# YuliangXiu/ICON

Hardware: NVIDIA H100
Metric: M query-points/sec at 256^3 grid (higher is better)
Workload: dtype f32

## Files before the change

### icon_b200/csrc/common.cuh

```cuda
#pragma once
#include <cuda_runtime.h>
#include <stdint.h>
#include <stdio.h>

#include "../../include/icon_b200.h"

namespace icon {

void set_error(const char *fmt, ...);
void count_launch(int n = 1);

#define ICON_CHECK_ARG(cond, ...)                 \
    do {                                          \
        if (!(cond)) {                            \
            icon::set_error(__VA_ARGS__);         \
            return ICON_EINVAL;                   \
        }                                         \
    } while (0)

#define ICON_CUDA(expr)                                                              \
    do {                                                                             \
        cudaError_t _e = (expr);                                                     \
        if (_e != cudaSuccess) {                                                     \
            icon::set_error("%s:%d %s -> %s", __FILE__, __LINE__, #expr,             \
// ... 124 lines not shown
    int nlevels;
    int lvl_cnt[TREE_MAX_LEVELS];
    int lvl_off[TREE_MAX_LEVELS];
};

struct MeshView : FaceTree {
    const float4 *tri;
    const float4 *sph;
    const float4 *attr;
    const float4 *rbox;
    float *vnormals;
    void *vn_ws;
    unsigned long long *keys;
    int32_t *rcount;
    int32_t *roff;
    int32_t *rlist;
    MeshHeader *hdr;
    void *scan_ws;
    float4 *bxyz;
    int32_t *bperm;
    float *brec;
    int32_t *bface;
    float *bub;
    int32_t *foff;
    unsigned short *flist;
    float *fkey;
    int64_t face_cap;
    int V;
};
size_t mesh_ws_bytes(int V, int F);
MeshView mesh_view(const void *ws, int V, int F);
void bricks_forget(const MeshView &m);

void profile_mark(int i, cudaStream_t stream);

size_t scan_ws_bytes(int64_t n);
int scan_exclusive_i32(const int32_t *in, int32_t *out, int64_t n, int64_t *d_total ,
                       void *ws, cudaStream_t stream);

struct CsrWs {
    int32_t *cnt, *cursor;
    void *scan_ws;
};
CsrWs csr_take(Carver &c, int64_t rows);
int csr_build(const int32_t *own, const int32_t *key, int64_t n, int R, int32_t *off, int32_t *list, int32_t *ucnt,
              const CsrWs &w, cudaStream_t stream);

size_t vertex_corners_ws_bytes(int V, int F);
int vertex_corners(const int64_t *faces, int F, int V, int32_t *off, int32_t *list, void *ws, cudaStream_t stream);

template <class Fn>
__device__ __forceinline__ void for_each_pass_corner(const int32_t *corners, int n, Fn &&fn) {
    for (int pass = 0; pass < 3; ++pass) {
        const int c = (pass + 1) % 3;
        for (int i = 0; i < n; ++i)
            if (corners[i] % 3 == c) fn(corners[i] / 3, c);
    }
}

size_t area_vertex_normals_ws_bytes(int V, int F);
int area_vertex_normals(const float *verts, int V, const int64_t *faces, int F, float *out, void *ws,
                        cudaStream_t stream);

}
```

### icon_b200/csrc/mlp.cu

```cuda
#include "common.cuh"
#include "query_common.cuh"

namespace icon {

constexpr int MP = 64;
constexpr int MT = 256;
constexpr int KC = 16;

constexpr int OFF_W0 = 0;
constexpr int OFF_B0 = OFF_W0 + 16 * 512;
constexpr int OFF_W1 = OFF_B0 + 512;
constexpr int OFF_B1 = OFF_W1 + 512 * 256;
constexpr int OFF_W2 = OFF_B1 + 256;
constexpr int OFF_B2 = OFF_W2 + 272 * 128;
constexpr int OFF_W3 = OFF_B2 + 128;
constexpr int OFF_B3 = OFF_W3 + 144;
static_assert(OFF_B3 + 1 == ICON_MLP_PACKED_FLOATS, "packed layout");

template <int MODE>
__global__ void __launch_bounds__(MT, 2) k_query_mlp(QueryParams q) {
    extern __shared__ __align__(16) float sm[];
    float *x0s = sm;
    float *stage = sm + 16 * MP;
    float *h1s = stage + 10240;
// ... 9 lines not shown

    {
        const float4 *src = (const float4 *)(W + OFF_W1);
        for (int i = tid; i < KC * 256 / 4; i += MT) cp_async16(w1c + 4 * i, src + i);
        cp_async_commit();
    }

    {
        const int pl = tid & (MP - 1), grp = tid >> 6;
        const int64_t pi = p0 + pl;
        const bool live = pi < q.N;
        if (MODE == 3) {
            for (int r = grp; r < 16; r += 4) x0s[r * MP + pl] = (live && r < c0) ? q.raw[(size_t)r * q.N + pi] : 0.f;
        } else {
            float4 xyz = live ? q.xyz4[pi] : make_float4(0.f, 0.f, 0.f, 0.f);
            if (MODE == 0) {
                const bool has_vis = q.feats & ICON_FEAT_VIS;
                const int d = has_vis ? q.C / 2 : q.C;
                float4 r0 = make_float4(0.f, 0.f, 0.f, 0.f), r1 = r0;
                if (live) {
                    const float4 *r = (const float4 *)(q.rec + 8 * pi);
                    r0 = r[0]; r1 = r[1];
                }
                const float vis = r1.w;
                if (grp == 0) {
                    float sdf = r0.x, cx = r0.y, cy = r0.z, cz = r0.w;
                    const bool outlier = live && fabsf(sdf) >= q.clip;
                    if (outlier) sdf = sdf > 0.f ? 1.f : -1.f;
                    int col = d;
                    x0s[col++ * MP + pl] = sdf;
                    if (q.feats & ICON_FEAT_CMAP) {
                        if (outlier) {
                            long long K = *q.d_K;
                            long long k3 = 3ll * (long long)q.krank[pi];
                            cx = (float)q.signs[(k3) % K];
                            cy = (float)q.signs[(k3 + 1) % K];
                            cz = (float)q.signs[(k3 + 2) % K];
                        }
                        x0s[col++ * MP + pl] = cx;
                        x0s[col++ * MP + pl] = cy;
                        x0s[col++ * MP + pl] = cz;
                    }
                    if (q.feats & ICON_FEAT_NORM) {
                        x0s[col++ * MP + pl] = r1.x;
                        x0s[col++ * MP + pl] = r1.y;
                        x0s[col++ * MP + pl] = r1.z;
                    }
                    for (int r = col; r < 16; ++r) x0s[r * MP + pl] = 0.f;
                } else {
                    const int base = !has_vis || vis != 0.f ? 0 : d;
                    for (int ch = grp - 1; ch < d; ch += 3) {
                        float v = live ? bilinear(q.feat + (size_t)(base + ch) * q.H * q.W, q.H, q.W, xyz.x, xyz.y) : 0.f;
                        x0s[ch * MP + pl] = v;
                    }
                }
            } else if (MODE == 1) {
                for (int ch = grp; ch < q.C; ch += 4) {
                    float v = live ? bilinear(q.feat + (size_t)ch * q.H * q.W, q.H, q.W, xyz.x, xyz.y) : 0.f;
                    x0s[ch * MP + pl] = v;
                }
                if (grp == 0) {
                    x0s[q.C * MP + pl] = live ? xyz.z : 0.f;
                    for (int r = q.C + 1; r < 16; ++r) x0s[r * MP + pl] = 0.f;
                }
            } else {
                if (grp < 3) {
                    for (int ch = grp; ch < q.C; ch += 3) {
// ... 119 lines not shown
        const int ch = ty * 4 + i;
        const float bia = __ldg(W + OFF_B2 + ch), w3 = __ldg(W + OFF_W3 + ch);
#pragma unroll
        for (int j = 0; j < 8; ++j) part[j] = fmaf(w3, lrelu(acc2[i][j] + bia), part[j]);
    }
#pragma unroll
    for (int j = 0; j < 8; ++j) {
        part[j] += __shfl_xor_sync(0xffffffffu, part[j], 8);
        part[j] += __shfl_xor_sync(0xffffffffu, part[j], 16);
    }
    const int lane = tid & 31, wid = tid >> 5;
    if (lane < 8) {
#pragma unroll
        for (int j = 0; j < 4; ++j) {
            red[wid * MP + lane * 4 + j] = part[j];
            red[wid * MP + 32 + lane * 4 + j] = part[4 + j];
        }
    }
    __syncthreads();
    if (tid < MP) {
        const int64_t pi = p0 + tid;
        if (pi < q.N) {
            float s = 0.f;
#pragma unroll
            for (int w = 0; w < 8; ++w) s += red[w * MP + tid];
            for (int j = 0; j < 16; ++j) s = fmaf(__ldg(W + OFF_W3 + 128 + j), x0s[j * MP + tid], s);
            s += __ldg(W + OFF_B3);
            float in_cube = (MODE == 3) ? 1.f : q.xyz4[pi].w;
            q.out[pi] = in_cube * s;
        }
    }
}

__global__ void k_outlier_flag(const float *__restrict__ rec, int64_t N, float clip, int32_t *__restrict__ flag) {
    int64_t i = (int64_t)blockIdx.x * blockDim.x + threadIdx.x;
    if (i < N) flag[i] = fabsf(rec[8 * i]) >= clip ? 1 : 0;
}
__global__ void k_outlier_signs(const float *__restrict__ rec, int64_t N, float clip,
                                const int32_t *__restrict__ krank, int8_t *__restrict__ signs) {
    int64_t i = (int64_t)blockIdx.x * blockDim.x + threadIdx.x;
    if (i < N) {
        float s = rec[8 * i];
        if (fabsf(s) >= clip) signs[krank[i]] = s > 0.f ? 1 : -1;
    }
}

constexpr size_t MLP_SMEM = (16 * MP + 10240 + 256 * MP) * sizeof(float);

template <int MODE>
static int launch_mlp(const QueryParams &q, cudaStream_t stream) {
    static bool attr_set[ICON_MAX_DEVICES] = {};
    if (device_needs_setup(attr_set))
        ICON_CUDA(cudaFuncSetAttribute(k_query_mlp<MODE>, cudaFuncAttributeMaxDynamicSharedMemorySize, (int)MLP_SMEM));
    unsigned nblk = (unsigned)((q.N + MP - 1) / MP);
    k_query_mlp<MODE><<<nblk, MT, MLP_SMEM, stream>>>(q);
    ICON_LAUNCHED();
    return ICON_OK;
}

int launch_mlp_tc(int mode, const QueryParams &q, const void *blob, cudaStream_t stream);
static int g_mlp_impl = 1;

template <int MODE>
static int launch_any(const QueryParams &q, const void *tc, cudaStream_t stream) {
    if (g_mlp_impl == 1) {
        if (!tc) {
            set_error("icon_query / icon_mlp_only: the tensor-core MLP needs the packed tensor-core weight blob (mlp_tc == NULL); "
                      "pass it or select the FP32 kernel with icon_set_mlp_impl(0)");
            return ICON_EINVAL;
        }
        if (q.c0 > 15) {
            set_error("icon_query / icon_mlp_only: the tensor-core MLP takes c0 <= 15 input channels (got %d)", q.c0);
            return ICON_EINVAL;
        }
        return launch_mlp_tc(MODE, q, tc, stream);
    }
    return launch_mlp<MODE>(q, stream);
}

size_t sdf_ws_bytes(int64_t N);
int run_sdf(const float *points, int64_t sc, int64_t sn, int64_t N, const float *h_calib, const MeshView &m,
            float *rec, int32_t *face, void *ws, float4 **xyz4_out, cudaStream_t stream);
int run_points_only(const float *points, int64_t sc, int64_t sn, int64_t N, const float *h_calib,
                    float4 *xyz4, cudaStream_t stream);

struct QueryWs {
    void *sdf_ws;
    float *rec;
    int32_t *krank;
    int8_t *signs;
    int64_t *d_K;
    void *scan_ws;
    float4 *xyz4;
};

static QueryWs carve_query(Carver &c, int64_t N, int prior) {
    QueryWs w{};
    if (prior == ICON_PRIOR_ICON) {
        w.sdf_ws = c.take<char>(sdf_ws_bytes(N));
        w.rec = c.take<float>((size_t)N * 8);
        w.krank = c.take<int32_t>((size_t)N);
        w.signs = c.take<int8_t>((size_t)N);
        w.d_K = c.take<int64_t>(1);
        w.scan_ws = c.take<char>(scan_ws_bytes(N));
    } else {
        w.xyz4 = c.take<float4>((size_t)N);
    }
    return w;
}

}

using namespace icon;

extern "C" size_t icon_query_workspace_bytes(int64_t N, int F, int prior) {
    (void)F;
    Carver c(nullptr);
    carve_query(c, N, prior);
    return c.total();
}

extern "C" int icon_query(int prior, const float *points, int64_t stride_c, int64_t stride_n, int64_t N,
                          const float *h_calib, const float *feat, int C, int H, int W,
                          const float *vol_feat, int VD, const void *mesh_ws, int V, int F,
                          const float *mlp_packed, const void *mlp_tc, int c0, float sdf_clip, float *out,
                          void *ws, size_t ws_bytes, icon_stream_t stream) {
    return icon_query_feats(prior, points, stride_c, stride_n, N, h_calib, feat, C, H, W, vol_feat, VD, mesh_ws, V, F,
                            mlp_packed, mlp_tc, c0, sdf_clip, ICON_FEAT_ALL, out, ws, ws_bytes, stream);
}

extern "C" int icon_query_feats(int prior, const float *points, int64_t stride_c, int64_t stride_n, int64_t N,
                                const float *h_calib, const float *feat, int C, int H, int W,
                                const float *vol_feat, int VD, const void *mesh_ws, int V, int F,
                                const float *mlp_packed, const void *mlp_tc, int c0, float sdf_clip, int smpl_feats,
                                float *out, void *ws, size_t ws_bytes, icon_stream_t stream_) {
    cudaStream_t stream = (cudaStream_t)stream_;
    ICON_CHECK_ARG(N >= 0 && N < (int64_t)INT32_MAX, "icon_query: N=%lld out of range", (long long)N);
    if (N == 0) return ICON_OK;
    ICON_CHECK_ARG(points && h_calib && feat && mlp_packed && out && ws, "icon_query: null pointer");
    ICON_CHECK_ARG(((uintptr_t)mlp_tc & 15) == 0, "icon_query: mlp_tc must be 16-byte aligned");
    ICON_CHECK_ARG(c0 >= 1 && c0 <= 16, "icon_query: c0=%d unsupported (1..16)", c0);
    ICON_CHECK_ARG(H >= 2 && W >= 2, "icon_query: feature map %dx%d too small", H, W);
    {
        Carver c(nullptr);
        carve_query(c, N, prior);
        if (ws_bytes < c.total()) {
            set_error("icon_query: workspace %zu < %zu", ws_bytes, c.total());
            return ICON_ENOSPC;
        }
    }
    Carver c(ws);
    QueryWs w = carve_query(c, N, prior);
    QueryParams q{};
    q.feat = feat; q.C = C; q.H = H; q.W = W; q.vol = vol_feat; q.VD = VD;
    q.mlp = mlp_packed; q.c0 = c0; q.clip = sdf_clip; q.out = out; q.N = N;
    if (prior == ICON_PRIOR_ICON) {
        ICON_CHECK_ARG(mesh_ws && V > 0 && F > 0, "icon_query: icon prior needs a prepared body mesh");
        ICON_CHECK_ARG((smpl_feats & ~ICON_FEAT_ALL) == 0, "icon_query: smpl_feats mask %d has bits outside ICON_FEAT_ALL",
                       smpl_feats);
        const int cm = smpl_feats & ICON_FEAT_CMAP ? 1 : 0, nm = smpl_feats & ICON_FEAT_NORM ? 1 : 0;
        const bool vs = smpl_feats & ICON_FEAT_VIS;
        const int tail = 1 + 3 * cm + 3 * nm;
        ICON_CHECK_ARG((!vs || C % 2 == 0) && c0 == (vs ? C / 2 : C) + tail,
                       "icon_query: icon prior with smpl_feats mask %d expects c0 = %s + %d (C=%d c0=%d)", smpl_feats,
                       vs ? "C/2" : "C", tail, C, c0);
        q.feats = smpl_feats;
        MeshView m = mesh_view(mesh_ws, V, F);
        float4 *xyz4 = nullptr;
        int rc = run_sdf(points, stride_c, stride_n, N, h_calib, m, w.rec, nullptr, w.sdf_ws, &xyz4, stream);
        if (rc) return rc;
        if (cm) {
            unsigned nb = (unsigned)((N + 255) / 256);
            k_outlier_flag<<<nb, 256, 0, stream>>>(w.rec, N, sdf_clip, w.krank);
            ICON_LAUNCHED();
            rc = scan_exclusive_i32(w.krank, w.krank, N, w.d_K, w.scan_ws, stream);
            if (rc) return rc;
            k_outlier_signs<<<nb, 256, 0, stream>>>(w.rec, N, sdf_clip, w.krank, w.signs);
            ICON_LAUNCHED();
            q.krank = w.krank; q.signs = w.signs; q.d_K = w.d_K;
        }
        q.xyz4 = xyz4; q.rec = w.rec;
        profile_mark(3, stream);
        rc = launch_any<0>(q, mlp_tc, stream);
        profile_mark(4, stream);
        return rc;
    }
    profile_mark(0, stream);
    int rc = run_points_only(points, stride_c, stride_n, N, h_calib, w.xyz4, stream);
    if (rc) return rc;
    profile_mark(1, stream); profile_mark(2, stream); profile_mark(3, stream);
    q.xyz4 = w.xyz4;
    if (prior == ICON_PRIOR_PIFU) {
        ICON_CHECK_ARG(C + 1 == c0, "icon_query: pifu prior expects c0 = C + 1 (C=%d c0=%d)", C, c0);
        rc = launch_any<1>(q, mlp_tc, stream);
        profile_mark(4, stream);
        return rc;
    }
    if (prior == ICON_PRIOR_PAMIR) {
        ICON_CHECK_ARG(vol_feat && VD >= 2 && C + 7 == c0, "icon_query: pamir prior expects vol_feat and c0 = C + 7");
        rc = launch_any<2>(q, mlp_tc, stream);
        profile_mark(4, stream);
        return rc;
    }
    set_error("icon_query: unknown prior %d", prior);
    return ICON_EINVAL;
}

extern "C" int icon_set_mlp_impl(int impl) {
    ICON_CHECK_ARG(impl == 0 || impl == 1, "icon_set_mlp_impl: 0 (fp32) or 1 (tensor cores)");
    g_mlp_impl = impl;
    return ICON_OK;
}
// ... 12 lines not shown
```

### icon_b200/csrc/mlp_tc.cu

```cuda
#include <cuda_fp16.h>

#include "common.cuh"
#include "query_common.cuh"
#include "wgmma.cuh"

namespace icon {

constexpr int TC_THREADS = 384;
constexpr int TC_M = 128;
constexpr int NSTAGE = 4;
constexpr int STAGE_BYTES = 32768;
constexpr int STAGES_PER_TILE = 20;
static_assert(STAGES_PER_TILE % NSTAGE == 0 && NSTAGE % 2 == 0, "layer-1 hi / lo pairs must stay on stages (2i, 2i + 1)");
constexpr int GATHER_THREADS = 96;

constexpr int TCB_W0 = 0;
constexpr int TCB_W1 = 32768;
constexpr int TCB_W2 = TCB_W1 + 8 * 65536;
constexpr int TCB_W2T = TCB_W2 + 4 * 32768;
constexpr int TCB_F32 = TCB_W2T + 8192;
constexpr int TCB_F32_FLOATS = 512 + 256 + 128 + 144 + 4;
constexpr int TCB_BYTES = TCB_F32 + TCB_F32_FLOATS * 4;
static_assert(TCB_BYTES == ICON_MLP_TC_BYTES, "blob layout");

// ... 30 lines not shown
        }
    }
}

template <int MODE>
__device__ __forceinline__ void gather_point(const QueryParams &q, int64_t pi, float *xf) {
#pragma unroll
    for (int j = 0; j < 15; ++j) xf[j * TC_M] = 0.f;
    float in_cube = 1.f;
    if (pi < q.N) {
        if (MODE == 3) {
            const int c0 = q.c0;
#pragma unroll
            for (int j = 0; j < 15; ++j)
                if (j < c0) xf[j * TC_M] = q.raw[(size_t)j * q.N + pi];
        } else {
            const float4 xyz = q.xyz4[pi];
            in_cube = xyz.w;
            if (MODE == 0) {
                const bool has_vis = q.feats & ICON_FEAT_VIS;
                const int d = has_vis ? q.C / 2 : q.C;
                const float4 *rp = (const float4 *)(q.rec + 8 * pi);
                const float4 r0 = rp[0], r1 = rp[1];
                const int fb = has_vis && r1.w == 0.f ? d : 0;
                float sdf = r0.x;
                const bool outlier = fabsf(sdf) >= q.clip;
                if (outlier) sdf = sdf > 0.f ? 1.f : -1.f;
                float *col = xf + d * TC_M;
                col[0] = sdf;
                col += TC_M;
                if (q.feats & ICON_FEAT_CMAP) {
                    float cx = r0.y, cy = r0.z, cz = r0.w;
                    if (outlier) {
                        const long long K = *q.d_K, k3 = 3ll * (long long)q.krank[pi];
                        cx = (float)q.signs[k3 % K];
                        cy = (float)q.signs[(k3 + 1) % K];
                        cz = (float)q.signs[(k3 + 2) % K];
                    }
                    col[0] = cx; col[TC_M] = cy; col[2 * TC_M] = cz;
                    col += 3 * TC_M;
                }
                if (q.feats & ICON_FEAT_NORM) { col[0] = r1.x; col[TC_M] = r1.y; col[2 * TC_M] = r1.z; }
                if (d == 6) {
#pragma unroll
                    for (int ch = 0; ch < 6; ++ch)
                        xf[ch * TC_M] = bilinear(q.feat + (size_t)(fb + ch) * q.H * q.W, q.H, q.W, xyz.x, xyz.y);
                } else {
#pragma unroll
                    for (int ch = 0; ch < 14; ++ch)
                        if (ch < d) xf[ch * TC_M] = bilinear(q.feat + (size_t)(fb + ch) * q.H * q.W, q.H, q.W, xyz.x, xyz.y);
                }
            } else if (MODE == 1) {
                if (q.C == 12) {
#pragma unroll
                    for (int ch = 0; ch < 12; ++ch)
                        xf[ch * TC_M] = bilinear(q.feat + (size_t)ch * q.H * q.W, q.H, q.W, xyz.x, xyz.y);
                } else {
#pragma unroll
                    for (int ch = 0; ch < 14; ++ch)
                        if (ch < q.C) xf[ch * TC_M] = bilinear(q.feat + (size_t)ch * q.H * q.W, q.H, q.W, xyz.x, xyz.y);
                }
                if (q.C < 15) xf[q.C * TC_M] = xyz.z;
            } else {
                const size_t vs = (size_t)q.VD * q.VD * q.VD;
                if (q.C == 6) {
#pragma unroll
                    for (int ch = 0; ch < 6; ++ch)
// ... 247 lines not shown
```

### icon_b200/csrc/query_common.cuh

```cuda
#pragma once
#include "common.cuh"

namespace icon {

struct QueryParams {
    const float4 *xyz4;
    const float *rec;
    const int32_t *krank;
    const int8_t *signs;
    const int64_t *d_K;
    int feats;
    const float *feat;
    int C, H, W;
    const float *vol;
    int VD;
    const float *raw;
    const float *mlp;
    int c0;
    float clip;
    float *out;
    int64_t N;
};

__device__ __forceinline__ float lrelu(float x) { return x > 0.f ? x : 0.01f * x; }

__device__ __forceinline__ void cp_async16(void *smem, const void *gmem) {
    unsigned s = (unsigned)__cvta_generic_to_shared(smem);
    asm volatile("cp.async.cg.shared.global [%0], [%1], 16;\n" ::"r"(s), "l"(gmem));
}
__device__ __forceinline__ void cp_async_commit() { asm volatile("cp.async.commit_group;\n" ::); }
template <int N>
__device__ __forceinline__ void cp_async_wait() { asm volatile("cp.async.wait_group %0;\n" ::"n"(N)); }

__device__ __forceinline__ float bilinear(const float *__restrict__ plane, int H, int W, float x, float y) {
    float ix = ((x + 1.f) / 2.f) * (float)(W - 1);
    float iy = ((y + 1.f) / 2.f) * (float)(H - 1);
    float fx = floorf(ix), fy = floorf(iy);
    int x0 = (int)fx, y0 = (int)fy, x1 = x0 + 1, y1 = y0 + 1;
    float wx1 = ix - fx, wy1 = iy - fy, wx0 = (fx + 1.f) - ix, wy0 = (fy + 1.f) - iy;
    float o = 0.f;
    bool vx0 = x0 >= 0 && x0 < W, vx1 = x1 >= 0 && x1 < W, vy0 = y0 >= 0 && y0 < H, vy1 = y1 >= 0 && y1 < H;
    if (vx0 && vy0) o += __ldg(plane + (size_t)y0 * W + x0) * (wx0 * wy0);
    if (vx1 && vy0) o += __ldg(plane + (size_t)y0 * W + x1) * (wx1 * wy0);
    if (vx0 && vy1) o += __ldg(plane + (size_t)y1 * W + x0) * (wx0 * wy1);
    if (vx1 && vy1) o += __ldg(plane + (size_t)y1 * W + x1) * (wx1 * wy1);
    return o;
}

__device__ __forceinline__ float trilinear(const float *__restrict__ v, int D, float x, float y, float z) {
    float ix = ((x + 1.f) / 2.f) * (float)(D - 1);
    float iy = ((y + 1.f) / 2.f) * (float)(D - 1);
    float iz = ((z + 1.f) / 2.f) * (float)(D - 1);
    float fx = floorf(ix), fy = floorf(iy), fz = floorf(iz);
    int x0 = (int)fx, y0 = (int)fy, z0 = (int)fz;
    float tx = ix - fx, ty = iy - fy, tz = iz - fz;
// ... 18 lines not shown
```

### icon_b200/csrc/sdf.cu

```cuda
#include <float.h>

#include <algorithm>
#include <mutex>
#include <type_traits>
#include <unordered_set>

#include "common.cuh"
#include "face_tree.cuh"
#include "geom.cuh"

namespace icon {

struct Calib {
    float r[9];
    float t[3];
};

__device__ __forceinline__ V3 load_point(const float *__restrict__ pts, int64_t sc, int64_t sn,
                                         int64_t i, const Calib &cb) {
    float px = pts[i * sn], py = pts[sc + i * sn], pz = pts[2 * sc + i * sn];
    V3 o;
    o.x = fmaf(cb.r[2], pz, fmaf(cb.r[1], py, cb.r[0] * px)) + cb.t[0];
    o.y = fmaf(cb.r[5], pz, fmaf(cb.r[4], py, cb.r[3] * px)) + cb.t[1];
    o.z = fmaf(cb.r[8], pz, fmaf(cb.r[7], py, cb.r[6] * px)) + cb.t[2];
    return o;
}

__device__ __forceinline__ void emit_record(V3 p, int bi, float best, int hits, const MeshView &m,
                                            float *__restrict__ rec, int32_t *__restrict__ face,
                                            int64_t idx) {
    Tri t = load_tri(m.tri + 3 * (size_t)bi);
    V3 n = cross3(t.ab, t.ac);
    float s = n.x * n.x + n.y * n.y + n.z * n.z;
    if (s == 0.f) s = 1e-6f;
    float inv = 1.0f / s;
    V3 w = sub3(p, t.a);
    V3 uw = cross3(t.ab, w), wv = cross3(w, t.ac);
    float b2 = (uw.x * n.x + uw.y * n.y + uw.z * n.z) * inv;
    float b1 = (wv.x * n.x + wv.y * n.y + wv.z * n.z) * inv;
    float b0 = 1.0f - b1 - b2;
    const float4 *at = m.attr + 6 * (size_t)bi;
    float4 a0 = __ldg(at), a1 = __ldg(at + 1), a2 = __ldg(at + 2), a3 = __ldg(at + 3),
           a4 = __ldg(at + 4), a5 = __ldg(at + 5);
    float nx = (a0.x * b0 + a0.w * b1 + a1.z * b2) * -1.f;
    float ny = (a0.y * b0 + a1.x * b1 + a1.w * b2) * 1.f;
    float nz = (a0.z * b0 + a1.y * b1 + a2.x * b2) * -1.f;
    float cx = a2.y * b0 + a3.x * b1 + a3.w * b2;
    float cy = a2.z * b0 + a3.y * b1 + a4.x * b2;
    float cz = a2.w * b0 + a3.z * b1 + a4.y * b2;
    float vv = a4.z * b0 + a4.w * b1 + a5.x * b2;
    float vis = vv >= 0.1f ? 1.f : 0.f;
    float dist = sqrtf(best) / sqrtf(3.0f);
    float sign = 2.0f * ((float)(hits & 1) - 0.5f);
    float sdf = dist * sign;
    float4 *r = (float4 *)(rec + 8 * idx);
    r[0] = make_float4(sdf, cx, cy, cz);
    r[1] = make_float4(nx, ny, nz, vis);
    if (face) face[idx] = bi;
}

constexpr int SW_T = 128;
constexpr int NBIN_AX = 128;
constexpr int NBIN = NBIN_AX * NBIN_AX * NBIN_AX;
__host__ __device__ constexpr int fr_cap(int ppw) { return ppw >= 16 ? 1024 : (ppw >= 4 ? 768 : 384); }

__device__ __forceinline__ unsigned spread7(unsigned v) {
    v = (v | (v << 16)) & 0x030000FFu;
    v = (v | (v << 8)) & 0x0300F00Fu;
    v = (v | (v << 4)) & 0x030C30C3u;
    v = (v | (v << 2)) & 0x09249249u;
    return v;
}

__device__ __forceinline__ int bin_of(V3 p) {
    const bool inside = p.x >= -1.f && p.x <= 1.f && p.y >= -1.f && p.y <= 1.f && p.z >= -1.f && p.z <= 1.f;
    if (!inside) return NBIN;
    const unsigned bx = min(NBIN_AX - 1, (int)((p.x + 1.f) * (NBIN_AX * 0.5f)));
    const unsigned by = min(NBIN_AX - 1, (int)((p.y + 1.f) * (NBIN_AX * 0.5f)));
    const unsigned bz = min(NBIN_AX - 1, (int)((p.z + 1.f) * (NBIN_AX * 0.5f)));
    return (int)(spread7(bx) | (spread7(by) << 1) | (spread7(bz) << 2));
}

__global__ void k_points_bin(const float *__restrict__ pts, int64_t sc, int64_t sn, int64_t N, Calib cb,
                             float4 *__restrict__ xyz4, int32_t *__restrict__ bid, int32_t *__restrict__ count) {
    const int64_t i = (int64_t)blockIdx.x * blockDim.x + threadIdx.x;
    const bool live = i < N;
    int b = -1;
    if (live) {
        const V3 p = load_point(pts, sc, sn, i, cb);
        const float in_cube = (p.x > -1.f && p.x < 1.f && p.y > -1.f && p.y < 1.f && p.z > -1.f && p.z < 1.f) ? 1.f : 0.f;
        xyz4[i] = make_float4(p.x, p.y, p.z, in_cube);
// ... 31 lines not shown
#define STAT(i, v) do { if (lane == 0) atomicAdd(&g_stats[i], (unsigned long long)(v)); } while (0)
#define WSTAT(i, v) do { if (lane == 0 && g_wstat) g_wstat[(size_t)wid * WS_N + (i)] = (unsigned)(v); } while (0)
#define WCLK(t) __syncwarp(); const long long t = clock64()
#else
#define STAT(i, v) do { } while (0)
#define WSTAT(i, v) do { } while (0)
#endif

template <int PPW, bool BRICK>
using SdfSmem = typename std::conditional<BRICK, ChunkSmem, WalkSmem<unsigned short, fr_cap(PPW)>>::type;
template <int PPW, bool BRICK>
constexpr size_t sdf_smem_bytes() { return sizeof(SdfSmem<PPW, BRICK>) * (SW_T / 32); }

constexpr float BRICK_W = 2.0f / BRICK_AX;
constexpr float BRICK_HALF_DIAG = 0.0541266f;

__device__ __forceinline__ void brick_box(int b, float4 &lo, float4 &hi) {
    const int bx = b % BRICK_AX, by = (b / BRICK_AX) % BRICK_AX, bz = b / (BRICK_AX * BRICK_AX);
    lo = make_float4(-1.f + bx * BRICK_W, -1.f + by * BRICK_W, -1.f + bz * BRICK_W, 0.f);
    hi = make_float4(-1.f + (bx + 1) * BRICK_W, -1.f + (by + 1) * BRICK_W, -1.f + (bz + 1) * BRICK_W, 0.f);
}

__device__ __forceinline__ float leaf_key(const MeshView &m, int l, float4 lo, float4 hi) {
    const float4 a = __ldg(m.nodes + 2 * (size_t)l), z = __ldg(m.nodes + 2 * (size_t)l + 1);
    const float gx = fmaxf(fmaxf(a.x - hi.x, lo.x - z.x), 0.f);
    const float gy = fmaxf(fmaxf(a.y - hi.y, lo.y - z.y), 0.f);
    const float gz = fmaxf(fmaxf(a.z - hi.z, lo.z - z.z), 0.f);
    return fmaf(gz, gz, fmaf(gy, gy, gx * gx));
}

template <int PPW, bool BRICK>
__device__ __forceinline__ void sdf_warp(int64_t wid, SdfSmem<PPW, BRICK> &S, const float4 *__restrict__ xyz4,
                                         const int32_t *__restrict__ perm, int64_t N, const MeshView &m,
                                         float *__restrict__ rec, int32_t *__restrict__ face,
                                         int32_t *__restrict__ defer, int32_t *__restrict__ ndefer) {
    constexpr int REP = 32 / PPW;
    const int lane = threadIdx.x & 31;
    const int sub = lane % PPW, rep_id = lane / PPW;
    const int64_t pos0 = wid * PPW;
    const int64_t pos = pos0 + sub;
    if (pos0 >= N) return;
    const bool live = pos < N;
    const int64_t idx = perm[live ? pos : pos0];
    const float4 q = xyz4[idx];
    const V3 p = mk3(q.x, q.y, q.z);
    const V3 c = mk3(0.5f * (warp_min(p.x) + warp_max(p.x)), 0.5f * (warp_min(p.y) + warp_max(p.y)),
                     0.5f * (warp_min(p.z) + warp_max(p.z)));
    const float rw = warp_max(sqrtf(dot3(sub3(p, c), sub3(p, c)))) * 1.00001f + 1e-6f;
    const float4 wlo = make_float4(warp_min(p.x) - 1e-6f, warp_min(p.y) - 1e-6f, warp_min(p.z) - 1e-6f, 0.f);
    const float4 whi = make_float4(warp_max(p.x) + 1e-6f, warp_max(p.y) + 1e-6f, warp_max(p.z) + 1e-6f, 0.f);
    const MeshHeader h = *m.hdr;

    NearestFace<PPW> nf(p, 1e-6f, 1e-7f);
#ifdef ICON_SDF_STATS
    WCLK(t_start);
    long long t_c = 0, t_ray = 0;
    int st_entries = 0, st_steps = 0, st_brick = -1;
    float st_ub0 = 0.f;
#endif
    if constexpr (BRICK) {
        bool ok = h.brick_built && !h.brick_overflow && c.x >= -1.f && c.x < 1.f && c.y >= -1.f && c.y < 1.f &&
                  c.z >= -1.f && c.z < 1.f;
        int b = 0;
        float4 blo, bhi;
        if (ok) {
            const int bx = min(BRICK_AX - 1, (int)((c.x + 1.f) * (BRICK_AX * 0.5f)));
            const int by = min(BRICK_AX - 1, (int)((c.y + 1.f) * (BRICK_AX * 0.5f)));
// ... 41 lines not shown
    WCLK(t_c1);
    int st_ray = 0;
#endif
    int hits = 0;
    if (!h.ray_overflow) {
        const float fy = (p.y - h.y0) * h.inv_cy, fz = (p.z - h.z0) * h.inv_cz;
        if (fy >= 0.f && fy < (float)RAY_GRID && fz >= 0.f && fz < (float)RAY_GRID) {
            const int cc = (int)fz * RAY_GRID + (int)fy;
            const int k0 = __ldg(m.roff + cc), k1 = __ldg(m.roff + cc + 1);
            for (int k = k0 + rep_id; k < k1; k += REP) {
                const int f = __ldg(m.rlist + k);
                if (__ldg(&m.rbox[2 * (size_t)f + 1].x) < p.x - 1e-3f) continue;
                const Tri tr = load_tri(m.tri + 3 * (size_t)f);
                hits += ray_hit_px(p, tr.a, tr.ab, tr.ac);
#ifdef ICON_SDF_STATS
                ++st_ray;
#endif
            }
        }
    } else {
        for (int f = rep_id; f < m.F; f += REP) {
            const Tri tr = load_tri(m.tri + 3 * (size_t)f);
            hits += ray_hit_px(p, tr.a, tr.ab, tr.ac);
        }
    }
    if (REP > 1) {
#pragma unroll
        for (int o = PPW; o < 32; o <<= 1) hits += __shfl_xor_sync(0xffffffffu, hits, o);
    }
#ifdef ICON_SDF_STATS
    WCLK(t_ray0);
    t_ray = t_ray0;
#endif
    if (live && rep_id == 0) emit_record(p, nf.bi, nf.best, hits, m, rec, face, idx);
#ifdef ICON_SDF_STATS
    WCLK(t_end);
    if (BRICK && st_brick >= 0) {
        const float ube = nf.ub;
        int il = 0, ifc = 0;
        const int o0 = __ldg(m.foff + st_brick), o1 = __ldg(m.foff + st_brick + 1);
        for (int s = o0 + lane; s < o1; s += 32) {
            il += __ldg(m.fkey + s) <= ube * ube;
            const float4 s4 = __ldg(m.sph_s + __ldg(m.flist + s));
            const float l2 = ube + s4.w;
            ifc += box_dist2(mk3(s4.x, s4.y, s4.z), wlo, whi) <= l2 * l2;
        }
        const int s_sph = __reduce_add_sync(0xffffffffu, nf.n_sph), s_exact = __reduce_add_sync(0xffffffffu, nf.n_exact);
        const int s_win = __reduce_add_sync(0xffffffffu, nf.n_win), s_ray = __reduce_add_sync(0xffffffffu, st_ray);
        const int s_il = __reduce_add_sync(0xffffffffu, il), s_if = __reduce_add_sync(0xffffffffu, ifc);
        WSTAT(WS_ENTRIES, st_entries);
        WSTAT(WS_STEPS, st_steps);
        WSTAT(WS_STAGED, nf.staged);
        WSTAT(WS_SPH, s_sph);
        WSTAT(WS_EXACT, s_exact);
        WSTAT(WS_WIN, s_win);
        WSTAT(WS_RAY, s_ray);
        WSTAT(WS_CYC_START, t_c - t_start);
        WSTAT(WS_CYC_C, t_c1 - t_c);
        WSTAT(WS_CYC_RAY, t_ray - t_c1);
        WSTAT(WS_CYC_EMIT, t_end - t_ray);
        WSTAT(WS_UB0, __float_as_uint(st_ub0));
        WSTAT(WS_UBEND, __float_as_uint(ube));
        WSTAT(WS_LIST, o1 - o0);
        WSTAT(WS_IDEAL_ENTRIES, s_il);
        WSTAT(WS_IDEAL_FACES, s_if);
        WSTAT(WS_DEAD, nf.n_dead);
    }
    if (!BRICK && defer != nullptr) { STAT(4, 1); STAT(5, t_end - t_start); }
#endif
}

template <int PPW, bool BRICK>
__global__ void __launch_bounds__(SW_T, PPW == 32 ? 8 : 0) k_sdf_warp(const float4 *__restrict__ xyz4, const int32_t *__restrict__ perm,
                                                   int64_t N, MeshView m, float *__restrict__ rec,
                                                   int32_t *__restrict__ face, int32_t *__restrict__ defer,
                                                   int32_t *__restrict__ ndefer) {
    static_assert(!BRICK || PPW == 32, "brick lists serve dense lattices: 32 points per warp");
    extern __shared__ __align__(16) unsigned char smem_raw[];
    SdfSmem<PPW, BRICK> &S = reinterpret_cast<SdfSmem<PPW, BRICK> *>(smem_raw)[threadIdx.x >> 5];
    const bool listed = !BRICK && defer != nullptr;
    const int64_t nw = listed ? (int64_t)*ndefer : (N + PPW - 1) / PPW;
    for (int64_t i = (int64_t)blockIdx.x * (SW_T / 32) + (threadIdx.x >> 5); i < nw; i += (int64_t)gridDim.x * (SW_T / 32))
        sdf_warp<PPW, BRICK>(listed ? (int64_t)defer[i] : i, S, xyz4, perm, N, m, rec, face, defer, ndefer);
}

__global__ void k_brick_centres(MeshView m) {
    const int b = blockIdx.x * blockDim.x + threadIdx.x;
    if (b >= NBRICK) return;
    float4 lo, hi;
    brick_box(b, lo, hi);
    m.bxyz[b] = make_float4(0.5f * (lo.x + hi.x), 0.5f * (lo.y + hi.y), 0.5f * (lo.z + hi.z), 0.f);
    m.bperm[b] = b;
}

template <class Take, class Put>
__device__ __forceinline__ int block_gather(int n, int *s_n, Take &&take, Put &&put) {
    __syncthreads();
    for (int i = threadIdx.x; i < n; i += blockDim.x) {
        float key;
        int tag;
        if (take(i, key, tag)) put(atomicAdd(s_n, 1), key, tag);
    }
    __syncthreads();
    return *s_n;
}

__device__ __forceinline__ unsigned long long key_tag(float key, int tag) {
    return (unsigned long long)__float_as_uint(key) << 32 | (unsigned)tag;
}

template <class Put>
__device__ __forceinline__ void rank_sort(const unsigned long long *s_kt, int n, Put &&put) {
    for (int i = threadIdx.x; i < n; i += blockDim.x) {
        const unsigned long long x = s_kt[i];
        int r = 0;
        for (int j = 0; j < n; ++j) r += s_kt[j] < x;
// ... 138 lines not shown
static std::mutex g_brick_mu;
static std::unordered_set<const void *> g_brick_ready;
static int64_t g_brick_builds = 0;

void bricks_forget(const MeshView &m) {
    std::lock_guard<std::mutex> lk(g_brick_mu);
    g_brick_ready.erase(m.hdr);
}

struct SdfWs {
    float4 *xyz4;
    int32_t *bid, *perm, *count, *offset;
    int32_t *defer, *ndefer;
    void *scan_ws;
};
static SdfWs carve_sdf(Carver &c, int64_t N) {
    SdfWs w;
    w.xyz4 = c.take<float4>((size_t)N);
    w.bid = c.take<int32_t>((size_t)N);
    w.perm = c.take<int32_t>((size_t)N);
    w.count = c.take<int32_t>(NBIN + 1);
    w.offset = c.take<int32_t>(NBIN + 1);
    w.defer = c.take<int32_t>((size_t)(N + 31) / 32);
    w.ndefer = c.take<int32_t>(1);
    w.scan_ws = c.take<char>(scan_ws_bytes(NBIN + 1));
    return w;
}

static int build_bricks(const MeshView &m, cudaStream_t stream) {
    const int64_t fcap = g_brick_max_entries > 0 ? std::min(g_brick_max_entries, m.face_cap) : m.face_cap;
    k_brick_centres<<<NBRICK / 256, 256, 0, stream>>>(m);
    ICON_LAUNCHED();
    k_sdf_warp<1, false><<<NBRICK / (SW_T / 32), SW_T, sdf_smem_bytes<1, false>(), stream>>>(
        m.bxyz, m.bperm, NBRICK, m, m.brec, m.bface, nullptr, nullptr);
    ICON_LAUNCHED();
    k_brick_faces<false><<<NBRICK, 128, 0, stream>>>(m, fcap);
    ICON_LAUNCHED();
    const int rc = scan_exclusive_i32(m.foff, m.foff, NBRICK + 1, nullptr, m.scan_ws, stream);
    if (rc) return rc;
    k_brick_faces<true><<<NBRICK, 128, 0, stream>>>(m, fcap);
    ICON_LAUNCHED();
    k_brick_done<<<1, 1, 0, stream>>>(m, fcap);
    ICON_LAUNCHED();
    return ICON_OK;
}
size_t sdf_ws_bytes(int64_t N) {
    Carver c(nullptr);
    carve_sdf(c, N);
    return c.total();
}

Calib make_calib(const float *h) {
    Calib cb;
    for (int r = 0; r < 3; ++r) {
        for (int k = 0; k < 3; ++k) cb.r[3 * r + k] = h[4 * r + k];
        cb.t[r] = h[4 * r + 3];
    }
    return cb;
}

int run_sdf(const float *points, int64_t sc, int64_t sn, int64_t N, const float *h_calib,
            const MeshView &m, float *rec, int32_t *face, void *ws, float4 **xyz4_out,
            cudaStream_t stream) {
    Carver c(ws);
    SdfWs w = carve_sdf(c, N);
    Calib cb = make_calib(h_calib);
    profile_mark(0, stream);
    ICON_CUDA(cudaMemsetAsync(w.count, 0, sizeof(int32_t) * (NBIN + 1), stream));
    const unsigned nblk = (unsigned)((N + 255) / 256);
    k_points_bin<<<nblk, 256, 0, stream>>>(points, sc, sn, N, cb, w.xyz4, w.bid, w.count);
    ICON_LAUNCHED();
    int rc = scan_exclusive_i32(w.count, w.offset, NBIN + 1, nullptr, w.scan_ws, stream);
    if (rc) return rc;
    ICON_CUDA(cudaMemsetAsync(w.count, 0, sizeof(int32_t) * (NBIN + 1), stream));
    k_points_scatter<<<nblk, 256, 0, stream>>>(w.bid, N, w.offset, w.count, w.perm);
    ICON_LAUNCHED();
    static bool attr_set[ICON_MAX_DEVICES] = {};
    if (device_needs_setup(attr_set)) {
#define ICON_SDF_ATTR(P, B) ICON_CUDA(cudaFuncSetAttribute(k_sdf_warp<P, B>, cudaFuncAttributeMaxDynamicSharedMemorySize, \
                                                           (int)sdf_smem_bytes<P, B>()))
        ICON_SDF_ATTR(32, true); ICON_SDF_ATTR(32, false); ICON_SDF_ATTR(16, false); ICON_SDF_ATTR(8, false);
        ICON_SDF_ATTR(4, false); ICON_SDF_ATTR(2, false); ICON_SDF_ATTR(1, false);
#undef ICON_SDF_ATTR
    }
    profile_mark(1, stream);
    int ppw = N >= g_sdf_ppw32_from ? 32 : (N >= g_sdf_ppw8_from ? 8 : 1);
    if (g_sdf_ppw_force) ppw = g_sdf_ppw_force;
    const int wpb = SW_T / 32;
    const int64_t nwarps = (N + ppw - 1) / ppw;
    const unsigned nblk_w = (unsigned)((nwarps + wpb - 1) / wpb);
#define ICON_SDF_LAUNCH(P) k_sdf_warp<P, false><<<nblk_w, SW_T, sdf_smem_bytes<P, false>(), stream>>>( \
        w.xyz4, w.perm, N, m, rec, face, nullptr, nullptr)
    if (ppw == 32 && g_sdf_bricks) {
        bool build;
        {
            std::lock_guard<std::mutex> lk(g_brick_mu);
            build = g_brick_ready.insert(m.hdr).second;
        }
        if (build) {
            rc = build_bricks(m, stream);
            std::lock_guard<std::mutex> lk(g_brick_mu);
            if (rc) { g_brick_ready.erase(m.hdr); return rc; }
            ++g_brick_builds;
        }
        ICON_CUDA(cudaMemsetAsync(w.ndefer, 0, sizeof(int32_t), stream));
        k_sdf_warp<32, true><<<nblk_w, SW_T, sdf_smem_bytes<32, true>(), stream>>>(
            w.xyz4, w.perm, N, m, rec, face, w.defer, w.ndefer);
        ICON_LAUNCHED();
        const unsigned nblk_d = (unsigned)std::min<int64_t>(nblk_w, (int64_t)device_sm_count() * 16);
        k_sdf_warp<32, false><<<nblk_d, SW_T, sdf_smem_bytes<32, false>(), stream>>>(
            w.xyz4, w.perm, N, m, rec, face, w.defer, w.ndefer);
    } else {
        switch (ppw) {
            case 32: ICON_SDF_LAUNCH(32); break;
            case 16: ICON_SDF_LAUNCH(16); break;
            case 8: ICON_SDF_LAUNCH(8); break;
            case 4: ICON_SDF_LAUNCH(4); break;
            case 2: ICON_SDF_LAUNCH(2); break;
            default: ICON_SDF_LAUNCH(1); break;
        }
    }
#undef ICON_SDF_LAUNCH
    ICON_LAUNCHED();
    profile_mark(2, stream);
    if (xyz4_out) *xyz4_out = w.xyz4;
    return ICON_OK;
}

__global__ void k_points_only(const float *__restrict__ pts, int64_t sc, int64_t sn, int64_t N, Calib cb,
                              float4 *__restrict__ xyz4) {
    int64_t i = (int64_t)blockIdx.x * blockDim.x + threadIdx.x;
    if (i >= N) return;
    V3 p = load_point(pts, sc, sn, i, cb);
    float in_cube = (p.x > -1.f && p.x < 1.f && p.y > -1.f && p.y < 1.f && p.z > -1.f && p.z < 1.f) ? 1.f : 0.f;
    xyz4[i] = make_float4(p.x, p.y, p.z, in_cube);
}

int run_points_only(const float *points, int64_t sc, int64_t sn, int64_t N, const float *h_calib,
                    float4 *xyz4, cudaStream_t stream) {
    Calib cb = make_calib(h_calib);
    k_points_only<<<(unsigned)((N + 255) / 256), 256, 0, stream>>>(points, sc, sn, N, cb, xyz4);
    ICON_LAUNCHED();
    return ICON_OK;
}
// ... 31 lines not shown
}

extern "C" int icon_sdf_brick_info(const void *mesh_ws, int V, int F, int64_t *out) {
    ICON_CHECK_ARG(mesh_ws && out && V > 0 && F > 0, "icon_sdf_brick_info: bad argument");
    MeshView m = mesh_view(mesh_ws, V, F);
    MeshHeader h;
    int32_t total = 0;
    ICON_CUDA(cudaDeviceSynchronize());
    ICON_CUDA(cudaMemcpy(&h, m.hdr, sizeof(h), cudaMemcpyDeviceToHost));
    if (h.brick_built) ICON_CUDA(cudaMemcpy(&total, m.foff + NBRICK, sizeof(total), cudaMemcpyDeviceToHost));
    out[0] = h.brick_built;
    out[1] = h.brick_overflow;
    out[2] = total;
    out[3] = m.face_cap;
    {
        std::lock_guard<std::mutex> lk(icon::g_brick_mu);
        out[4] = icon::g_brick_builds;
    }
    return ICON_OK;
}

extern "C" int icon_sdf_only(const float *points, int64_t stride_c, int64_t stride_n, int64_t N,
                             const float *h_calib, const void *mesh_ws, int V, int F, float *rec,
                             int32_t *face, void *ws, size_t ws_bytes, icon_stream_t stream_) {
    cudaStream_t stream = (cudaStream_t)stream_;
    ICON_CHECK_ARG(N >= 0 && N < (int64_t)INT32_MAX, "icon_sdf_only: N=%lld out of range", (long long)N);
    if (N == 0) return ICON_OK;
    ICON_CHECK_ARG(points && h_calib && mesh_ws && rec && ws, "icon_sdf_only: null pointer");
    if (ws_bytes < sdf_ws_bytes(N)) {
        set_error("icon_sdf_only: workspace %zu < %zu", ws_bytes, sdf_ws_bytes(N));
        return ICON_ENOSPC;
    }
    MeshView m = mesh_view(mesh_ws, V, F);
    return run_sdf(points, stride_c, stride_n, N, h_calib, m, rec, face, ws, nullptr, stream);
}

extern "C" int icon_sdf_bruteforce(const float *points, int64_t stride_c, int64_t stride_n, int64_t N,
                                   const float *h_calib, const void *mesh_ws, int V, int F, float *rec,
                                   int32_t *face, icon_stream_t stream_) {
    cudaStream_t stream = (cudaStream_t)stream_;
    if (N == 0) return ICON_OK;
    ICON_CHECK_ARG(points && h_calib && mesh_ws && rec, "icon_sdf_bruteforce: null pointer");
    MeshView m = mesh_view(mesh_ws, V, F);
    Calib cb = make_calib(h_calib);
    k_sdf_brute<<<(unsigned)((N + 255) / 256), 256, 0, stream>>>(points, stride_c, stride_n, N, cb, m, rec, face);
    ICON_LAUNCHED();
    return ICON_OK;
}
```

Measured before the change: 635.7.

## Fuse outlier flagging into SDF kernel and compact ranks via warp bitmasks

Result: no change. 642.2 (median of 6 runs) (+1.0%).

```diff
diff --git a/icon_b200/csrc/common.cuh b/icon_b200/csrc/common.cuh
--- a/icon_b200/csrc/common.cuh
+++ b/icon_b200/csrc/common.cuh
@@ -180,6 +180,11 @@
 MeshView mesh_view(const void *ws, int V, int F);
 void bricks_forget(const MeshView &m);
 
+struct OutlierFlags {
+    uint8_t *flag;
+    float clip;
+};
+
 void profile_mark(int i, cudaStream_t stream);
 
 size_t scan_ws_bytes(int64_t n);
diff --git a/icon_b200/csrc/mlp.cu b/icon_b200/csrc/mlp.cu
--- a/icon_b200/csrc/mlp.cu
+++ b/icon_b200/csrc/mlp.cu
@@ -65,7 +65,7 @@
                     if (q.feats & ICON_FEAT_CMAP) {
                         if (outlier) {
                             long long K = *q.d_K;
-                            long long k3 = 3ll * (long long)q.krank[pi];
+                            long long k3 = 3ll * outlier_rank(q, pi);
                             cx = (float)q.signs[(k3) % K];
                             cy = (float)q.signs[(k3 + 1) % K];
                             cz = (float)q.signs[(k3 + 2) % K];
@@ -251,17 +251,23 @@
     }
 }
 
-__global__ void k_outlier_flag(const float *__restrict__ rec, int64_t N, float clip, int32_t *__restrict__ flag) {
-    int64_t i = (int64_t)blockIdx.x * blockDim.x + threadIdx.x;
-    if (i < N) flag[i] = fabsf(rec[8 * i]) >= clip ? 1 : 0;
-}
-__global__ void k_outlier_signs(const float *__restrict__ rec, int64_t N, float clip,
-                                const int32_t *__restrict__ krank, int8_t *__restrict__ signs) {
-    int64_t i = (int64_t)blockIdx.x * blockDim.x + threadIdx.x;
-    if (i < N) {
-        float s = rec[8 * i];
-        if (fabsf(s) >= clip) signs[krank[i]] = s > 0.f ? 1 : -1;
-    }
+__global__ void k_outlier_pack(const uint8_t *__restrict__ flag, int64_t N, int64_t nw, unsigned *__restrict__ out_bits,
+                               unsigned *__restrict__ pos_bits, int32_t *__restrict__ cnt) {
+    const int64_t i = (int64_t)blockIdx.x * blockDim.x + threadIdx.x, w = i >> 5;
+    const unsigned f = i < N ? flag[i] : 0u;
+    const unsigned o = __ballot_sync(0xffffffffu, f & 1u), s = __ballot_sync(0xffffffffu, f & 2u);
+    if ((i & 31) == 0 && w < nw) {
+        out_bits[w] = o;
+        pos_bits[w] = s;
+        cnt[w] = __popc(o);
+    }
+}
+__global__ void k_outlier_signs(const unsigned *__restrict__ out_bits, const unsigned *__restrict__ pos_bits, int64_t nw,
+                                const int32_t *__restrict__ wprefix, int8_t *__restrict__ signs) {
+    const int64_t i = (int64_t)blockIdx.x * blockDim.x + threadIdx.x, w = i >> 5;
+    if (w >= nw) return;
+    const unsigned bits = out_bits[w], bit = 1u << (i & 31);
+    if (bits & bit) signs[wprefix[w] + __popc(bits & (bit - 1u))] = pos_bits[w] & bit ? 1 : -1;
 }
 
 constexpr size_t MLP_SMEM = (16 * MP + 10240 + 256 * MP) * sizeof(float);
@@ -299,14 +305,16 @@
 
 size_t sdf_ws_bytes(int64_t N);
 int run_sdf(const float *points, int64_t sc, int64_t sn, int64_t N, const float *h_calib, const MeshView &m,
-            float *rec, int32_t *face, void *ws, float4 **xyz4_out, cudaStream_t stream);
+            float *rec, int32_t *face, const OutlierFlags &of, void *ws, float4 **xyz4_out, cudaStream_t stream);
 int run_points_only(const float *points, int64_t sc, int64_t sn, int64_t N, const float *h_calib,
                     float4 *xyz4, cudaStream_t stream);
 
 struct QueryWs {
     void *sdf_ws;
     float *rec;
-    int32_t *krank;
+    uint8_t *flag;
+    unsigned *bits;
+    int32_t *wprefix;
     int8_t *signs;
     int64_t *d_K;
     void *scan_ws;
@@ -316,12 +324,15 @@
 static QueryWs carve_query(Carver &c, int64_t N, int prior) {
     QueryWs w{};
     if (prior == ICON_PRIOR_ICON) {
+        const int64_t nw = (N + 31) / 32;
         w.sdf_ws = c.take<char>(sdf_ws_bytes(N));
         w.rec = c.take<float>((size_t)N * 8);
-        w.krank = c.take<int32_t>((size_t)N);
+        w.flag = c.take<uint8_t>((size_t)N);
+        w.bits = c.take<unsigned>(2 * (size_t)nw);
+        w.wprefix = c.take<int32_t>((size_t)nw);
         w.signs = c.take<int8_t>((size_t)N);
         w.d_K = c.take<int64_t>(1);
-        w.scan_ws = c.take<char>(scan_ws_bytes(N));
+        w.scan_ws = c.take<char>(scan_ws_bytes(nw));
     } else {
         w.xyz4 = c.take<float4>((size_t)N);
     }
@@ -386,17 +397,20 @@
         q.feats = smpl_feats;
         MeshView m = mesh_view(mesh_ws, V, F);
         float4 *xyz4 = nullptr;
-        int rc = run_sdf(points, stride_c, stride_n, N, h_calib, m, w.rec, nullptr, w.sdf_ws, &xyz4, stream);
+        const int64_t nw = (N + 31) / 32;
+        const OutlierFlags of{cm ? w.flag : nullptr, sdf_clip};
+        int rc = run_sdf(points, stride_c, stride_n, N, h_calib, m, w.rec, nullptr, of, w.sdf_ws, &xyz4, stream);
         if (rc) return rc;
         if (cm) {
-            unsigned nb = (unsigned)((N + 255) / 256);
-            k_outlier_flag<<<nb, 256, 0, stream>>>(w.rec, N, sdf_clip, w.krank);
+            unsigned *out_bits = w.bits, *pos_bits = w.bits + nw;
+            const unsigned nb = (unsigned)((nw + 7) / 8);
+            k_outlier_pack<<<nb, 256, 0, stream>>>(w.flag, N, nw, out_bits, pos_bits, w.wprefix);
             ICON_LAUNCHED();
-            rc = scan_exclusive_i32(w.krank, w.krank, N, w.d_K, w.scan_ws, stream);
+            rc = scan_exclusive_i32(w.wprefix, w.wprefix, nw, w.d_K, w.scan_ws, stream);
             if (rc) return rc;
-            k_outlier_signs<<<nb, 256, 0, stream>>>(w.rec, N, sdf_clip, w.krank, w.signs);
+            k_outlier_signs<<<nb, 256, 0, stream>>>(out_bits, pos_bits, nw, w.wprefix, w.signs);
             ICON_LAUNCHED();
-            q.krank = w.krank; q.signs = w.signs; q.d_K = w.d_K;
+            q.out_bits = out_bits; q.wprefix = w.wprefix; q.signs = w.signs; q.d_K = w.d_K;
         }
         q.xyz4 = xyz4; q.rec = w.rec;
         profile_mark(3, stream);
diff --git a/icon_b200/csrc/mlp_tc.cu b/icon_b200/csrc/mlp_tc.cu
--- a/icon_b200/csrc/mlp_tc.cu
+++ b/icon_b200/csrc/mlp_tc.cu
@@ -86,7 +86,7 @@
                 if (q.feats & ICON_FEAT_CMAP) {
                     float cx = r0.y, cy = r0.z, cz = r0.w;
                     if (outlier) {
-                        const long long K = *q.d_K, k3 = 3ll * (long long)q.krank[pi];
+                        const long long K = *q.d_K, k3 = 3ll * outlier_rank(q, pi);
                         cx = (float)q.signs[k3 % K];
                         cy = (float)q.signs[(k3 + 1) % K];
                         cz = (float)q.signs[(k3 + 2) % K];
diff --git a/icon_b200/csrc/query_common.cuh b/icon_b200/csrc/query_common.cuh
--- a/icon_b200/csrc/query_common.cuh
+++ b/icon_b200/csrc/query_common.cuh
@@ -6,7 +6,8 @@
 struct QueryParams {
     const float4 *xyz4;
     const float *rec;
-    const int32_t *krank;
+    const unsigned *out_bits;
+    const int32_t *wprefix;
     const int8_t *signs;
     const int64_t *d_K;
     int feats;
@@ -21,6 +22,10 @@
     float *out;
     int64_t N;
 };
+
+__device__ __forceinline__ long long outlier_rank(const QueryParams &q, int64_t pi) {
+    return (long long)q.wprefix[pi >> 5] + __popc(q.out_bits[pi >> 5] & ((1u << (pi & 31)) - 1u));
+}
 
 __device__ __forceinline__ float lrelu(float x) { return x > 0.f ? x : 0.01f * x; }
 
diff --git a/icon_b200/csrc/sdf.cu b/icon_b200/csrc/sdf.cu
--- a/icon_b200/csrc/sdf.cu
+++ b/icon_b200/csrc/sdf.cu
@@ -26,7 +26,7 @@
     return o;
 }
 
-__device__ __forceinline__ void emit_record(V3 p, int bi, float best, int hits, const MeshView &m,
+__device__ __forceinline__ float emit_record(V3 p, int bi, float best, int hits, const MeshView &m,
                                             float *__restrict__ rec, int32_t *__restrict__ face,
                                             int64_t idx) {
     Tri t = load_tri(m.tri + 3 * (size_t)bi);
@@ -57,6 +57,7 @@
     r[0] = make_float4(sdf, cx, cy, cz);
     r[1] = make_float4(nx, ny, nz, vis);
     if (face) face[idx] = bi;
+    return sdf;
 }
 
 constexpr int SW_T = 128;
@@ -154,7 +155,7 @@
 template <int PPW, bool BRICK>
 __device__ __forceinline__ void sdf_warp(int64_t wid, SdfSmem<PPW, BRICK> &S, const float4 *__restrict__ xyz4,
                                          const int32_t *__restrict__ perm, int64_t N, const MeshView &m,
-                                         float *__restrict__ rec, int32_t *__restrict__ face,
+                                         float *__restrict__ rec, int32_t *__restrict__ face, const OutlierFlags &of,
                                          int32_t *__restrict__ defer, int32_t *__restrict__ ndefer) {
     constexpr int REP = 32 / PPW;
     const int lane = threadIdx.x & 31;
@@ -262,7 +263,10 @@
     WCLK(t_ray0);
     t_ray = t_ray0;
 #endif
-    if (live && rep_id == 0) emit_record(p, nf.bi, nf.best, hits, m, rec, face, idx);
+    if (live && rep_id == 0) {
+        const float sdf = emit_record(p, nf.bi, nf.best, hits, m, rec, face, idx);
+        if (of.flag) of.flag[idx] = fabsf(sdf) >= of.clip ? (sdf > 0.f ? 3 : 1) : 0;
+    }
 #ifdef ICON_SDF_STATS
     WCLK(t_end);
     if (BRICK && st_brick >= 0) {
@@ -303,15 +307,15 @@
 template <int PPW, bool BRICK>
 __global__ void __launch_bounds__(SW_T, PPW == 32 ? 8 : 0) k_sdf_warp(const float4 *__restrict__ xyz4, const int32_t *__restrict__ perm,
                                                    int64_t N, MeshView m, float *__restrict__ rec,
-                                                   int32_t *__restrict__ face, int32_t *__restrict__ defer,
-                                                   int32_t *__restrict__ ndefer) {
+                                                   int32_t *__restrict__ face, OutlierFlags of,
+                                                   int32_t *__restrict__ defer, int32_t *__restrict__ ndefer) {
     static_assert(!BRICK || PPW == 32, "brick lists serve dense lattices: 32 points per warp");
     extern __shared__ __align__(16) unsigned char smem_raw[];
     SdfSmem<PPW, BRICK> &S = reinterpret_cast<SdfSmem<PPW, BRICK> *>(smem_raw)[threadIdx.x >> 5];
     const bool listed = !BRICK && defer != nullptr;
     const int64_t nw = listed ? (int64_t)*ndefer : (N + PPW - 1) / PPW;
     for (int64_t i = (int64_t)blockIdx.x * (SW_T / 32) + (threadIdx.x >> 5); i < nw; i += (int64_t)gridDim.x * (SW_T / 32))
-        sdf_warp<PPW, BRICK>(listed ? (int64_t)defer[i] : i, S, xyz4, perm, N, m, rec, face, defer, ndefer);
+        sdf_warp<PPW, BRICK>(listed ? (int64_t)defer[i] : i, S, xyz4, perm, N, m, rec, face, of, defer, ndefer);
 }
 
 __global__ void k_brick_centres(MeshView m) {
@@ -516,7 +520,7 @@
     k_brick_centres<<<NBRICK / 256, 256, 0, stream>>>(m);
     ICON_LAUNCHED();
     k_sdf_warp<1, false><<<NBRICK / (SW_T / 32), SW_T, sdf_smem_bytes<1, false>(), stream>>>(
-        m.bxyz, m.bperm, NBRICK, m, m.brec, m.bface, nullptr, nullptr);
+        m.bxyz, m.bperm, NBRICK, m, m.brec, m.bface, OutlierFlags{}, nullptr, nullptr);
     ICON_LAUNCHED();
     k_brick_faces<false><<<NBRICK, 128, 0, stream>>>(m, fcap);
     ICON_LAUNCHED();
@@ -544,7 +548,7 @@
 }
 
 int run_sdf(const float *points, int64_t sc, int64_t sn, int64_t N, const float *h_calib,
-            const MeshView &m, float *rec, int32_t *face, void *ws, float4 **xyz4_out,
+            const MeshView &m, float *rec, int32_t *face, const OutlierFlags &of, void *ws, float4 **xyz4_out,
             cudaStream_t stream) {
     Carver c(ws);
     SdfWs w = carve_sdf(c, N);
@@ -574,7 +578,7 @@
     const int64_t nwarps = (N + ppw - 1) / ppw;
     const unsigned nblk_w = (unsigned)((nwarps + wpb - 1) / wpb);
 #define ICON_SDF_LAUNCH(P) k_sdf_warp<P, false><<<nblk_w, SW_T, sdf_smem_bytes<P, false>(), stream>>>( \
-        w.xyz4, w.perm, N, m, rec, face, nullptr, nullptr)
+        w.xyz4, w.perm, N, m, rec, face, of, nullptr, nullptr)
     if (ppw == 32 && g_sdf_bricks) {
         bool build;
         {
@@ -589,11 +593,11 @@
         }
         ICON_CUDA(cudaMemsetAsync(w.ndefer, 0, sizeof(int32_t), stream));
         k_sdf_warp<32, true><<<nblk_w, SW_T, sdf_smem_bytes<32, true>(), stream>>>(
-            w.xyz4, w.perm, N, m, rec, face, w.defer, w.ndefer);
+            w.xyz4, w.perm, N, m, rec, face, of, w.defer, w.ndefer);
         ICON_LAUNCHED();
         const unsigned nblk_d = (unsigned)std::min<int64_t>(nblk_w, (int64_t)device_sm_count() * 16);
         k_sdf_warp<32, false><<<nblk_d, SW_T, sdf_smem_bytes<32, false>(), stream>>>(
-            w.xyz4, w.perm, N, m, rec, face, w.defer, w.ndefer);
+            w.xyz4, w.perm, N, m, rec, face, of, w.defer, w.ndefer);
     } else {
         switch (ppw) {
             case 32: ICON_SDF_LAUNCH(32); break;
@@ -691,7 +695,7 @@
         return ICON_ENOSPC;
     }
     MeshView m = mesh_view(mesh_ws, V, F);
-    return run_sdf(points, stride_c, stride_n, N, h_calib, m, rec, face, ws, nullptr, stream);
+    return run_sdf(points, stride_c, stride_n, N, h_calib, m, rec, face, OutlierFlags{}, ws, nullptr, stream);
 }
 
 extern "C" int icon_sdf_bruteforce(const float *points, int64_t stride_c, int64_t stride_n, int64_t N,
```
